# lazear/sage

Measured on NVIDIA H100. Metric: spectra/sec, higher is better.
Workload: dtype f32

## Files before the change

### sage_b200/csrc/device_common.cuh

```cuda
#pragma once
#include <cuda_runtime.h>
#include <stdint.h>

namespace sb {

constexpr int K_MAX = 128;
constexpr uint32_t NARROW_CAP = 8192;
constexpr int PRELIM_THREADS = 256;
constexpr int SCORE_THREADS = 128;
#ifndef SAGE_B200_SCORE_MIN_CTAS
#define SAGE_B200_SCORE_MIN_CTAS 10
#endif
constexpr int SCORE_MIN_CTAS = SAGE_B200_SCORE_MIN_CTAS;
#ifndef SAGE_B200_SCORE_TILE
#define SAGE_B200_SCORE_TILE 1024
#endif
#ifndef SAGE_B200_SCORE_UNROLL
#define SAGE_B200_SCORE_UNROLL 1
#endif
#ifndef SAGE_B200_SCORE_MIN_CTAS_SPLIT
#define SAGE_B200_SCORE_MIN_CTAS_SPLIT 11
#endif
constexpr int SCORE_MIN_CTAS_SPLIT = SAGE_B200_SCORE_MIN_CTAS_SPLIT;
constexpr uint32_t SCORE_UNROLL = SAGE_B200_SCORE_UNROLL;
// ... 158 lines not shown
    const uint32_t* bucket_lut;
    float blut_base, blut_inv_w;
    const uint32_t* pep_lut;
    float plut_base, plut_inv_w;
    uint64_t n_frag;
    uint8_t kinds[MAX_KINDS];
};

struct WideIndexView {
    const uint2* frag;
    const uint64_t* blk_off;
    const uint32_t* lut;
    uint32_t block, n_block, cells;
    float base, inv_w;
};

struct ScorerView {
    Tol precursor_tol, fragment_tol;
    uint32_t min_matched_peaks;
    int min_iso, max_iso;
    uint32_t min_charge, max_charge;
    int override_charge, max_fragment_charge_opt, chimera, wide_window, annotate, score_type;
    uint32_t report_psms;
    uint32_t kparam;
    uint32_t n_iso;
    uint32_t n_ch_max;
    uint32_t qmax;
    uint32_t lcap;
    uint32_t pep_cap;
    uint32_t wide_tile;
// ... 35 lines not shown
```

### sage_b200/csrc/kernels.cuh

```cuda
#pragma once
#include <type_traits>

#include "device_common.cuh"
#include "glibc_log.cuh"

#ifndef SAGE_B200_RARE_NOINLINE
#define SAGE_B200_RARE_NOINLINE 0
#endif
#if SAGE_B200_RARE_NOINLINE
#define SB_RARE __noinline__
#else
#define SB_RARE __forceinline__
#endif

namespace sb {

__device__ __forceinline__ uint32_t pep_partition(const DbView& db, float x, bool le) {
    uint32_t lo = 0, hi = db.n_pep;
    if (db.pep_lut != nullptr) {
        const float t = (x - db.plut_base) * db.plut_inv_w;
        if (t == t) {
            const int c = (int)fminf(fmaxf(floorf(t), -2.0f), (float)PEP_LUT_CELLS + 2.0f);
            lo = __ldg(db.pep_lut + min(max(c - 1, 0), (int)PEP_LUT_CELLS));
            hi = __ldg(db.pep_lut + min(max(c + 2, 0), (int)PEP_LUT_CELLS));
// ... 244 lines not shown
            const uint2 f = __ldg(&slice[e]);
            if (f.x > q.pre_hi) break;
            const float fmz = __uint_as_float(f.y);
            if (f.x >= q.eff_lo && f.x <= q.eff_hi && fmz >= flo && fmz <= fhi) {
                const uint32_t idx = f.x - q.pre_lo;
                atomicAdd(&cnt32[idx >> 1], 1u << ((idx & 1) * 16));
                matched++;
            }
        }
        pages++;
        entries += e - il;
    }
}

#ifndef SAGE_B200_WALK_SOLO
#define SAGE_B200_WALK_SOLO 8
#endif
constexpr uint32_t WALK_SOLO = SAGE_B200_WALK_SOLO;
__device__ __forceinline__ void block_probe_warp(const WideIndexView& nv, const QueryDesc& q, uint32_t b0, uint32_t b1, bool act, float flo, float fhi,
                                                 uint32_t* cnt32, uint32_t& matched) {
    const uint32_t lane = threadIdx.x & 31;
    const float tt = (flo - nv.base) * nv.inv_w;
    const int c = tt > 1.0f ? (int)fminf(tt, (float)(nv.cells - 1)) - 1 : 0;
    for (uint32_t blk = b0; blk <= b1; blk++) {
        const uint64_t base = __ldg(nv.blk_off + blk);
        const uint32_t cnt = (uint32_t)(__ldg(nv.blk_off + blk + 1) - base);
        const uint2* fr = nv.frag + base;
        uint32_t e = cnt;
        if (act) {
            e = __ldg(nv.lut + (size_t)blk * (nv.cells + 1) + c);
            for (uint32_t k = 0; k < WALK_SOLO && e < cnt; k++, e++) {
                const uint2 f = __ldg(fr + e);
                const float fmz = __uint_as_float(f.y);
                if (fmz > fhi) { e = cnt; break; }
                if (fmz >= flo && f.x >= q.eff_lo && f.x <= q.eff_hi) {
                    const uint32_t idx = f.x - q.pre_lo;
                    atomicAdd(&cnt32[idx >> 1], 1u << ((idx & 1) * 16));
                    matched++;
                }
            }
        }
        uint32_t pend = __ballot_sync(0xffffffffu, e < cnt);
        while (pend) {
            const int src = __ffs(pend) - 1;
            pend &= pend - 1;
            const uint32_t e0 = __shfl_sync(0xffffffffu, e, src);
            const float lo_s = __shfl_sync(0xffffffffu, flo, src), hi_s = __shfl_sync(0xffffffffu, fhi, src);
            for (uint32_t pos = e0; pos < cnt; pos += 32) {
                const uint32_t i = pos + lane;
                bool stop = i >= cnt;
                if (!stop) {
                    const uint2 f = __ldg(fr + i);
                    const float fmz = __uint_as_float(f.y);
                    stop = fmz > hi_s;
                    if (!stop && fmz >= lo_s && f.x >= q.eff_lo && f.x <= q.eff_hi) {
                        const uint32_t idx = f.x - q.pre_lo;
                        atomicAdd(&cnt32[idx >> 1], 1u << ((idx & 1) * 16));
                        matched++;
                    }
                }
                if (__any_sync(0xffffffffu, stop)) break;
            }
        }
    }
}

__device__ __forceinline__ void narrow_cta_query(const DbView& db, const ScorerView& sc, const BatchView& b, uint32_t pmax, uint64_t* nlist, uint32_t item,
                                                 float* bounds_smem, const WideIndexView& nv) {
    __shared__ uint32_t cnt32[NARROW_CAP / 2 + 1];
    __shared__ uint32_t s_warp[40];
    ReplaySlot* const nslots = b.nslots;
    const uint32_t s = item / sc.qmax;
    const QueryDesc q = b.queries[item];
    const uint32_t tid = threadIdx.x, lane = tid & 31, warp = tid >> 5, nwarps = PRELIM_THREADS / 32;
    const uint32_t p0 = b.peak_off[s], np = b.peak_off[s + 1] - p0;
    const uint32_t nwords = (q.potential + 1) >> 1;
    for (uint32_t i = tid; i < nwords; i += PRELIM_THREADS) cnt32[i] = 0;
    __shared__ unsigned long long s_loff;
    if (tid == 0 && q.potential > sc.kparam) s_loff = atomicAdd(b.counters + C_NLIST, (unsigned long long)q.potential);

    const uint32_t nfc = q.nfc;
    const uint32_t ntask = np * nfc;
    uint32_t my_matched = 0, my_pages = 0, my_entries = 0;
// ... 60 lines not shown
                                uint32_t bb = lut_start(LP, luts + (2 * c + 1) * LUT_CELLS, f);
                                while (bb < a && hi_c[bb] < f) bb++;
                                c_here += a - min(bb, a);
                            }
                        }
                    }
                }
                for (int o = 16; o > 0; o >>= 1) c_here += __shfl_down_sync(0xffffffffu, c_here, o);
                if (lane == 0 && c_here) {
                    const uint32_t idx = pep - q.pre_lo;
                    atomicAdd(&cnt32[idx >> 1], (c_here & 0xFFFFu) << ((idx & 1) * 16));
                    my_matched += c_here;
                }
            }
        }
    } else if (nv.frag != nullptr) {
        const uint32_t blk0 = q.pre_lo / nv.block, blk1 = min(q.pre_hi, db.n_pep - 1) / nv.block;
        for (uint32_t t0 = warp * 32; t0 < ntask; t0 += PRELIM_THREADS) {
            const uint32_t t = t0 + lane;
            const bool act = t < ntask;
            float flo = 0.0f, fhi = 0.0f;
            if (act) {
                const uint32_t p = t / nfc, fc = t - p * nfc + 1;
                const float mass = __fmul_rn(__ldg(b.masses + p0 + p), (float)fc);
                tol_bounds(sc.fragment_tol, mass, flo, fhi);
            }
            block_probe_warp(nv, q, blk0, blk1, act, flo, fhi, cnt32, my_matched);
        }
    } else {
        for (uint32_t t = tid; t < ntask; t += PRELIM_THREADS) {
            const uint32_t p = t / nfc, fc = t - p * nfc + 1;
// ... 77 lines not shown
            const uint32_t x = s_warp[w];
            if (w < warp) off += x;
            total += x;
        }
        if (c) list[wbase + off + __popc(ball & ((1u << lane) - 1))] = prescore_key(c, q.pre_lo + i, q.charge, q.iso);
        wbase += total;
        __syncthreads();
    }
    const uint32_t nzt = block_sum_u32(nzc, s_warp);
    if (tid == 0) {
        h->n = k; h->default_run = 0; h->matched_peaks = matched_total; h->scored_candidates = nzt;
        slot->off = loff; slot->item = item; slot->n_list = wbase; slot->state = 0; slot->k = k;
    }
}

__global__ void __launch_bounds__(PRELIM_THREADS) k_prelim_narrow(DbView db, ScorerView sc, BatchView b, uint32_t pmax, uint64_t* nlist, WideIndexView nv) {
    extern __shared__ float bounds_smem[];
    const uint32_t total = (uint32_t)min(b.counters[C_NCTA], (unsigned long long)b.n * sc.qmax);
    for (uint32_t i = blockIdx.x; i < total; i += gridDim.x) {
        narrow_cta_query(db, sc, b, pmax, nlist, b.cta_items[i], bounds_smem, nv);
        __syncthreads();
    }
}

template <bool BLK>
__global__ void __launch_bounds__(WARPQ_WARPS * 32, WARPQ_MIN_CTAS) k_prelim_narrow_warp(DbView db, ScorerView sc, BatchView b, uint64_t* nlist, uint32_t s_lo,
                                                                                                uint32_t s_hi, WideIndexView nv) {
    __shared__ uint32_t cnt_all[WARPQ_WARPS][WARPQ_CAP / 2];
    if (b.counters[C_COUNT + blockIdx.y] == 0ull) return;
    const uint32_t lane = threadIdx.x & 31, warp = threadIdx.x >> 5;
    const uint32_t pos = blockIdx.x * WARPQ_WARPS + warp;
    if (pos >= b.n) return;
    const uint32_t s = b.order ? b.order[pos] : pos;
    if (s < s_lo || s >= s_hi) return;
    const uint32_t item = s * sc.qmax + blockIdx.y;
    const QueryDesc q = b.queries[item];
    if (q.mode != 4) return;
    uint32_t* const cnt32 = cnt_all[warp];
    const uint32_t n = q.potential, k = min(n, sc.kparam);
    for (uint32_t i = lane; i < (n + 1) >> 1; i += 32) cnt32[i] = 0;
    unsigned long long loff = 0;
    if (n > k) {
// ... 1981 lines not shown
}
__global__ void k_wide_keys(uint64_t n_frag, const uint2* frag, uint32_t block, uint64_t* key64, uint32_t* pep) {
    const uint64_t i = (uint64_t)blockIdx.x * blockDim.x + threadIdx.x;
    if (i >= n_frag) return;
    const uint2 f = frag[i];
    key64[i] = ((uint64_t)(f.x / block) << 32) | (uint32_t)((uint32_t)f32_key(__uint_as_float(f.y)) ^ 0x80000000u);
    pep[i] = f.x;
}
__global__ void k_wide_pack(uint64_t n_frag, const uint64_t* key64, const uint32_t* pep, uint2* out) {
    const uint64_t i = (uint64_t)blockIdx.x * blockDim.x + threadIdx.x;
    if (i >= n_frag) return;
    const uint32_t u = (uint32_t)key64[i] ^ 0x80000000u;
    const uint32_t bits = u ^ (((uint32_t)((int)u >> 31)) >> 1);
    out[i] = make_uint2(pep[i], bits);
}
__global__ void k_wide_block_offsets(uint64_t n_frag, const uint64_t* key64, uint32_t n_block, uint64_t* blk_off) {
    const uint32_t b = blockIdx.x * blockDim.x + threadIdx.x;
    if (b > n_block) return;
    uint64_t lo = 0, hi = n_frag;
    const uint64_t want = (uint64_t)b << 32;
    while (lo < hi) { const uint64_t m = (lo + hi) >> 1; if (key64[m] < want) lo = m + 1; else hi = m; }
    blk_off[b] = lo;
}
__global__ void k_window_sample(DbView db, Tol ptol, uint32_t samples, unsigned long long* sum) {
    const uint32_t k = blockIdx.x * blockDim.x + threadIdx.x;
    if (k >= samples || db.n_pep == 0) return;
    const uint32_t i = (uint32_t)((uint64_t)k * db.n_pep / samples);
    float lo, hi;
    tol_bounds(ptol, __ldg(db.pep_mono + i), lo, hi);
    const uint32_t a = pep_partition(db, lo, false), b = pep_partition(db, hi, true);
    atomicAdd(sum, (unsigned long long)(b > a ? b - a : 0u));
}
__global__ void k_frag_mz_range(uint64_t n_frag, const uint2* frag, uint32_t* rng) {
    uint32_t lo = 0xFFFFFFFFu, hi = 0u;
    for (uint64_t i = (uint64_t)blockIdx.x * blockDim.x + threadIdx.x; i < n_frag; i += (uint64_t)gridDim.x * blockDim.x) {
        const uint32_t y = frag[i].y;
        lo = min(lo, y); hi = max(hi, y);
// ... 75 lines not shown
```

### sage_b200/csrc/sage_b200.cu

```cuda
#include <cub/device/device_radix_sort.cuh>
#include <cub/device/device_scan.cuh>
#include <cuda_runtime.h>

#include <pthread.h>
#include <sched.h>

#include <algorithm>
#include <atomic>
#include <cctype>
#include <cmath>
#include <cstdarg>
#include <cstdio>
#include <cstdlib>
#include <cstring>
#include <chrono>
#include <condition_variable>
#include <memory>
#include <mutex>
#include <thread>
#include <string>
#include <vector>

#include "../../include/sage_b200.h"
#include "kernels.cuh"
// ... 146 lines not shown
    const size_t nthreads = std::min<size_t>(max_threads, (size_t)hw - 1);
    const cudaError_t e = pool.run(dst, src, bytes, stage.p, piece, nthreads, st);
    if (e != cudaSuccess) return fail(SAGE_B200_ECUDA, "staged host-to-device copy failed: %s", cudaGetErrorString(e));
    return 0;
}

static bool is_pinned(const void* p) {
    cudaPointerAttributes a;
    if (cudaPointerGetAttributes(&a, p) != cudaSuccess) {
        cudaGetLastError();
        return false;
    }
    return a.type == cudaMemoryTypeHost;
}

struct BlockIndexSlot {
    WideIndexView v{};
    void *d_frag = nullptr, *d_blk = nullptr, *d_lut = nullptr;
    int failed = 0;
    uint64_t bytes = 0;
    std::vector<void*> retired;
    uint64_t retired_bytes = 0;
    void release() {
        for (void** p : {&d_frag, &d_blk, &d_lut}) { if (*p) cudaFree(*p); *p = nullptr; }
        for (void* p : retired) cudaFree(p);
        retired.clear();
        retired_bytes = 0;
        v = WideIndexView{};
        bytes = 0;
    }
    void retire() {
        for (void** p : {&d_frag, &d_blk, &d_lut}) { if (*p) retired.push_back(*p); *p = nullptr; }
        retired_bytes += bytes;
        v = WideIndexView{};
        bytes = 0;
    }
};

struct sage_b200_db {
    int device = 0;
    DbView v{};
    void *d_page_grid = nullptr, *d_bucket_lut = nullptr, *d_pep_lut = nullptr;
    void *d_frag = nullptr, *d_bucket_min = nullptr, *d_pep_mono = nullptr, *d_ion_off = nullptr, *d_ions = nullptr, *d_pep_len = nullptr,
         *d_pep_flags = nullptr, *d_pep_missed = nullptr;
    uint64_t total_residues = 0, device_bytes = 0;
    int sm_count = 132;
    mutable std::mutex wmu;
    mutable BlockIndexSlot wide, narrow;
};

static int dmalloc(sage_b200_db* db, void** p, size_t bytes) {
    if (bytes == 0) bytes = 16;
    CUDA_TRY(cudaMalloc(p, bytes));
    db->device_bytes += bytes;
    return 0;
}

static uint32_t ceil_log2_u64(uint64_t n) {
    uint32_t l = 0;
    while ((1ull << l) < n) l++;
    return l;
}

// ... 323 lines not shown
    if (nf && (fragment_peptide || fragment_mz)) {
        void *t_pep = nullptr, *t_mz = nullptr;
        CUDA_TRY(cudaMalloc(&t_pep, 4 * nf));
        CUDA_TRY(cudaMalloc(&t_mz, 4 * nf));
        k_unpack_fragments<<<(unsigned)((nf + 255) / 256), 256>>>(nf, db->v.frag, (uint32_t*)t_pep, (float*)t_mz);
        cudaError_t e = cudaDeviceSynchronize();
        if (e == cudaSuccess && fragment_peptide) e = cudaMemcpy(fragment_peptide, t_pep, 4 * nf, cudaMemcpyDeviceToHost);
        if (e == cudaSuccess && fragment_mz) e = cudaMemcpy(fragment_mz, t_mz, 4 * nf, cudaMemcpyDeviceToHost);
        cudaFree(t_pep); cudaFree(t_mz);
        if (e != cudaSuccess) return fail(SAGE_B200_ECUDA, "export failed: %s", cudaGetErrorString(e));
    }
    if (bucket_min && db->v.n_bucket) CUDA_TRY(cudaMemcpy(bucket_min, db->d_bucket_min, 4ull * db->v.n_bucket, cudaMemcpyDeviceToHost));
    return 0;
}

static WideIndexView build_block_index(const sage_b200_db* db, BlockIndexSlot& slot, uint32_t block, uint32_t cells) {
    WideIndexView none{};
    if (slot.v.frag != nullptr && slot.v.block == block) return slot.v;
    if (slot.failed || block == 0 || db->v.n_frag == 0 || db->v.n_pep == 0) return none;
    const uint64_t nf = db->v.n_frag;
    slot.retire();
    void *k_a = nullptr, *k_b = nullptr, *p_a = nullptr, *p_b = nullptr, *tmp = nullptr, *d_rng = nullptr;
    auto cleanup = [&]() { for (void* p : {k_a, k_b, p_a, p_b, tmp, d_rng}) if (p) cudaFree(p); };
    auto give_up = [&]() { cleanup(); for (void** p : {&slot.d_frag, &slot.d_blk, &slot.d_lut}) { if (*p) cudaFree(*p); *p = nullptr; } slot.v = WideIndexView{}; slot.bytes = 0; cudaGetLastError(); slot.failed = 1; return WideIndexView{}; };
    const uint32_t n_block = (db->v.n_pep + block - 1) / block;
    while (cells > 256 && (uint64_t)n_block * (cells + 1) * 4 > (1024ull << 20)) cells >>= 1;
    if (cudaMalloc(&slot.d_frag, 8 * nf + 64) != cudaSuccess || cudaMalloc(&slot.d_blk, 8 * ((size_t)n_block + 1)) != cudaSuccess ||
        cudaMalloc(&slot.d_lut, 4 * (size_t)n_block * (cells + 1)) != cudaSuccess)
        return give_up();
    if (cudaMalloc(&k_a, 8 * nf) != cudaSuccess || cudaMalloc(&k_b, 8 * nf) != cudaSuccess || cudaMalloc(&p_a, 4 * nf) != cudaSuccess ||
        cudaMalloc(&p_b, 4 * nf) != cudaSuccess || cudaMalloc(&d_rng, 8) != cudaSuccess)
        return give_up();
    k_wide_keys<<<(unsigned)((nf + 255) / 256), 256>>>(nf, db->v.frag, block, (uint64_t*)k_a, (uint32_t*)p_a);
    int nb_bits = 1;
    while (nb_bits < 32 && (n_block >> nb_bits)) nb_bits++;
    size_t tb = 0;
    if (nf > 0x7FFFFFFFull) return give_up();
    if (cub::DeviceRadixSort::SortPairs(nullptr, tb, (const uint64_t*)k_a, (uint64_t*)k_b, (const uint32_t*)p_a, (uint32_t*)p_b, (int)nf, 0, 32 + nb_bits) != cudaSuccess ||
        cudaMalloc(&tmp, tb + 16) != cudaSuccess ||
        cub::DeviceRadixSort::SortPairs(tmp, tb, (const uint64_t*)k_a, (uint64_t*)k_b, (const uint32_t*)p_a, (uint32_t*)p_b, (int)nf, 0, 32 + nb_bits) != cudaSuccess)
        return give_up();
    k_wide_pack<<<(unsigned)((nf + 255) / 256), 256>>>(nf, (const uint64_t*)k_b, (const uint32_t*)p_b, (uint2*)slot.d_frag);
    k_wide_block_offsets<<<(n_block + 1 + 255) / 256, 256>>>(nf, (const uint64_t*)k_b, n_block, (uint64_t*)slot.d_blk);
    const uint32_t rng0[2] = {0xFFFFFFFFu, 0u};
    if (cudaMemcpy(d_rng, rng0, 8, cudaMemcpyHostToDevice) != cudaSuccess) return give_up();
    k_frag_mz_range<<<(unsigned)std::min<uint64_t>((nf + 255) / 256, 4096), 256>>>(nf, db->v.frag, (uint32_t*)d_rng);
    uint32_t rng[2];
    if (cudaMemcpy(rng, d_rng, 8, cudaMemcpyDeviceToHost) != cudaSuccess) return give_up();
    cleanup();
    k_a = k_b = p_a = p_b = tmp = d_rng = nullptr;
    float lo, hi;
    memcpy(&lo, &rng[0], 4); memcpy(&hi, &rng[1], 4);
    WideIndexView w{};
    w.frag = (const uint2*)slot.d_frag; w.blk_off = (const uint64_t*)slot.d_blk; w.lut = (const uint32_t*)slot.d_lut;
    w.block = block; w.n_block = n_block; w.cells = cells;
    const float width = (hi - lo) / (float)cells;
    w.base = (std::isfinite(lo) && lo > 0.0f) ? lo : 0.0f;
    w.inv_w = (std::isfinite(width) && width > 0.0f && lo > 0.0f) ? 1.0f / width : 0.0f;
    if (w.inv_w > 0.0f) {
        const uint64_t total = (uint64_t)n_block * (cells + 1);
        k_wide_lut<<<(unsigned)((total + 255) / 256), 256>>>(w, (uint32_t*)slot.d_lut);
    } else if (cudaMemset(slot.d_lut, 0, 4 * (size_t)n_block * (cells + 1)) != cudaSuccess) return give_up();
    if (cudaDeviceSynchronize() != cudaSuccess) return give_up();
    slot.v = w;
    slot.bytes = 8 * nf + 8 * ((uint64_t)n_block + 1) + 4ull * n_block * (cells + 1);
    return w;
}

static WideIndexView db_wide_index(const sage_b200_db* db, uint32_t block) {
    std::lock_guard<std::mutex> lock(db->wmu);
    if (const char* e = getenv("SAGE_B200_NO_WIDE_INDEX")) if (e[0] == '1') return WideIndexView{};
    return build_block_index(db, db->wide, block, 1u << 18);
}

static WideIndexView db_narrow_index(const sage_b200_db* db, uint32_t block, uint32_t cells_x, bool exact) {
    std::lock_guard<std::mutex> lock(db->wmu);
    if (!exact && db->narrow.v.frag != nullptr && db->narrow.v.block * 2 >= block && db->narrow.v.block <= block * 2) return db->narrow.v;
    const uint32_t n_block = (db->v.n_pep + block - 1) / std::max(block, 1u);
    const uint64_t per_block = n_block ? db->v.n_frag / n_block : 0;
    uint32_t cells = 1024;
    while (cells < (1u << 18) && (uint64_t)cells < per_block * cells_x) cells <<= 1;
    return build_block_index(db, db->narrow, block, cells);
}

static int ensure_kernel_attributes(int device) {
    static std::mutex mu;
    static bool done[64] = {};
    std::lock_guard<std::mutex> lock(mu);
    if (device >= 0 && device < 64 && done[device]) return 0;
    int optin = 0;
    CUDA_TRY(cudaDeviceGetAttribute(&optin, cudaDevAttrMaxSharedMemoryPerBlockOptin, device));
    auto raise = [&](const void* fn) -> cudaError_t {
        cudaFuncAttributes fa;
        cudaError_t e = cudaFuncGetAttributes(&fa, fn);
        if (e != cudaSuccess) return e;
        return cudaFuncSetAttribute(fn, cudaFuncAttributeMaxDynamicSharedMemorySize, optin - (int)fa.sharedSizeBytes);
    };
// ... 115 lines not shown
    ScorerView sv{};
    std::mutex mu;
    Lane lanes[2];
    DevBuf d_lnfact, d_keep;
    uint32_t quick_mode = 0;
    int sort_spectra = 1;
    sage_b200_fragment* frag_dst = nullptr;
    uint64_t frag_cap = 0, frag_used = 0;
    int pipeline_chunks = 1;
    double nlist_per_spectrum = 512.0, wide_per_spectrum = 0.0;
    int score_split = 1;
    double hits_per_spectrum = 0.0;
    int narrow_index = 1;
    uint32_t narrow_block_auto = 0;
    int narrow_cta = 1;
    uint32_t narrow_block = 0 , narrow_cells_x = 4;
    int mass_parts = 2;
    int first_chunk_pct = 0;
    bool trace = false;
    cudaEvent_t ev_base = nullptr;
    std::chrono::steady_clock::time_point t_base;
    sage_b200_counters last{};
};

extern "C" int sage_b200_scorer_create(const sage_b200_db* db, const sage_b200_scorer_params* p, sage_b200_scorer** out) {
    if (!db || !p || !out) return fail(SAGE_B200_EINVAL, "scorer_create: null argument");
    if (p->report_psms == 0) return fail(SAGE_B200_EINVAL, "report_psms must be >= 1");
    if (p->report_psms > K_MAX / 2) return fail(SAGE_B200_ELIMIT, "report_psms %u > %d not supported", p->report_psms, K_MAX / 2);
    if (p->precursor_tol.kind < 0 || p->precursor_tol.kind > 2 || p->fragment_tol.kind < 0 || p->fragment_tol.kind > 2) return fail(SAGE_B200_EINVAL, "bad tolerance kind");
    if (p->score_type > 1) return fail(SAGE_B200_EINVAL, "bad score_type");
    CUDA_TRY(cudaSetDevice(db->device));
// ... 46 lines not shown
        CUDA_TRY(cudaStreamCreateWithFlags(&L.stream, cudaStreamNonBlocking));
        CUDA_TRY(cudaStreamCreateWithFlags(&L.copy, cudaStreamNonBlocking));
        for (auto& e : L.ev) CUDA_TRY(cudaEventCreate(&e));
        CUDA_TRY(cudaEventCreate(&L.ev_masses));
        CUDA_TRY(cudaEventCreate(&L.ev_intens));
        CUDA_TRY(cudaEventCreate(&L.ev_small));
        for (auto& e : L.ev_part) CUDA_TRY(cudaEventCreate(&e));
        CUDA_TRY(cudaStreamCreateWithFlags(&L.copy2, cudaStreamNonBlocking));
    }
    if (const char* e = getenv("SAGE_B200_PIPELINE_CHUNKS")) s->pipeline_chunks = std::max(1, atoi(e));
    if (const char* e = getenv("SAGE_B200_TRACE")) s->trace = e[0] == '1';
    if (const char* e = getenv("SAGE_B200_SCORE_SPLIT")) s->score_split = atoi(e) != 0;
    if (const char* e = getenv("SAGE_B200_NARROW_INDEX")) s->narrow_index = atoi(e) != 0;
    if (const char* e = getenv("SAGE_B200_NARROW_CTA")) s->narrow_cta = atoi(e) != 0;
    if (const char* e = getenv("SAGE_B200_NARROW_BLOCK")) s->narrow_block = (uint32_t)std::max(0, atoi(e));
    if (const char* e = getenv("SAGE_B200_NARROW_CELLS_X")) s->narrow_cells_x = (uint32_t)std::max(1, atoi(e));
    if (const char* e = getenv("SAGE_B200_MASS_PARTS")) s->mass_parts = std::min(MASS_PARTS, std::max(1, atoi(e)));
    if (const char* e = getenv("SAGE_B200_FIRST_CHUNK_PCT")) s->first_chunk_pct = std::min(50, std::max(0, atoi(e)));
    CUDA_TRY(cudaEventCreate(&s->ev_base));
    *out = s;
    return 0;
}

extern "C" int sage_b200_scorer_set_option(sage_b200_scorer* s, const char* name, int64_t value) {
    if (!s || !name) return fail(SAGE_B200_EINVAL, "scorer_set_option: null argument");
    std::lock_guard<std::mutex> lock(s->mu);
    if (!strcmp(name, "sort_spectra")) { s->sort_spectra = value != 0; return 0; }
    if (!strcmp(name, "pipeline_chunks")) { s->pipeline_chunks = (int)std::max<int64_t>(1, value); return 0; }
    if (!strcmp(name, "score_split")) { s->score_split = value != 0; return 0; }
    if (!strcmp(name, "narrow_index")) { s->narrow_index = value != 0; return 0; }
    if (!strcmp(name, "narrow_block")) {
        if (value != 0 && (value < 64 || value > (1 << 20))) return fail(SAGE_B200_EINVAL, "narrow_block must be 0 (automatic) or 64..1048576");
        s->narrow_block = (uint32_t)value;
        return 0;
    }
    if (!strcmp(name, "mass_parts")) {
        if (value < 1 || value > MASS_PARTS) return fail(SAGE_B200_EINVAL, "mass_parts must be 1..%d", MASS_PARTS);
        s->mass_parts = (int)value;
        return 0;
    }
    if (!strcmp(name, "wide_lmax")) {
        if (value < (int64_t)K_MAX || value > (int64_t)WIDE_LMAX) return fail(SAGE_B200_EINVAL, "wide_lmax must be in %d..%u", K_MAX, WIDE_LMAX);
        s->sv.wide_lmax = (uint32_t)value;
        return 0;
    }
    if (!strcmp(name, "wide_tile")) {
        if (value < 256 || value > (int64_t)WIDE_TILE || (value & 1)) return fail(SAGE_B200_EINVAL, "wide_tile must be even and in 256..%u", WIDE_TILE);
// ... 267 lines not shown
    bv.wide_cap = C.wide_cap;
    bv.nlist_cap = C.nlist_cap;
    k_setup_queries<<<(n + 127) / 128, 128, 0, st>>>(db->v, svq, bv, sk_in, sv_in);
    CUDA_TRY(cudaGetLastError());
    if (sk_in) {
        CUDA_TRY(cub::DeviceRadixSort::SortPairs(L.d_sorttmp.p, sort_tmp, sk_in, sk_out, sv_in, sv_out, (int)n, sort_lo, sort_bits, st));
        bv.order = sv_out;
    }
    CUDA_TRY(cudaEventRecord(L.ev[2], st));
    if (C.nparts <= 1) CUDA_TRY(cudaStreamWaitEvent(st, L.ev_masses, 0));
    uint64_t launches = 1;

    const size_t rsm = (size_t)sv.kparam * REPLAY_THREADS * 8;
    const float ptol_span = std::max(std::fabs(sv.precursor_tol.lo), std::fabs(sv.precursor_tol.hi));
    const bool narrow_tol = ptol_span <= (sv.precursor_tol.kind == 0 ? 2000.0f : sv.precursor_tol.kind == 1 ? 0.2f : 5.0f);
    WideIndexView nv{};
    if (S->narrow_index && !sv.wide_window && narrow_tol) {
        if (S->narrow_block == 0 && (rc = narrow_block_for(S))) return rc;
        nv = db_narrow_index(db, S->narrow_block ? S->narrow_block : S->narrow_block_auto, S->narrow_cells_x, S->narrow_block != 0);
    }
    for (uint32_t q = 0; q < C.nparts; q++) {
        if (C.nparts > 1) CUDA_TRY(cudaStreamWaitEvent(st, L.ev_part[q], 0));
        const dim3 wgrid((n + WARPQ_WARPS - 1) / WARPQ_WARPS, sv.qmax);
        if (nv.frag != nullptr) k_prelim_narrow_warp<true><<<wgrid, WARPQ_WARPS * 32, 0, st>>>(db->v, svq, bv, L.d_nlist.as<uint64_t>(), C.part_lo[q], C.part_lo[q + 1], nv);
        else k_prelim_narrow_warp<false><<<wgrid, WARPQ_WARPS * 32, 0, st>>>(db->v, svq, bv, L.d_nlist.as<uint64_t>(), C.part_lo[q], C.part_lo[q + 1], nv);
        CUDA_TRY(cudaGetLastError());
        launches += q > 0;
    }
    if (C.nparts > 1) CUDA_TRY(cudaStreamWaitEvent(st, L.ev_masses, 0));
    k_prelim_narrow<<<(unsigned)std::min<uint64_t>(C.nitems, (uint64_t)db->sm_count * 6), PRELIM_THREADS, pep_smem, st>>>(db->v, svq, bv, C.pmax, L.d_nlist.as<uint64_t>(),
                                                                                                                         S->narrow_cta ? nv : WideIndexView{});
    CUDA_TRY(cudaGetLastError());
    CUDA_TRY(cudaEventRecord(L.ev[8], st));
    k_replay<true><<<(unsigned)((C.nitems + REPLAY_THREADS - 1) / REPLAY_THREADS), REPLAY_THREADS, rsm / 2, st>>>(sv, bv, L.d_nlist.as<uint64_t>(), L.d_nslots.as<ReplaySlot>(),
                                                                                                                 (uint32_t)C.nitems, nullptr, n);
    CUDA_TRY(cudaGetLastError());
    launches += 3;
    if (C.wide_cap) {
        const int ctas = (int)std::min<uint64_t>((uint64_t)db->sm_count * WIDE_CTAS, C.wide_cap);
        const WideIndexView wv = db_wide_index(db, sv.wide_tile);
        k_prelim_wide<<<ctas, WIDE_THREADS, sizeof(WideSmem), st>>>(db->v, sv, bv, (uint32_t)C.nitems, L.d_wlist.as<uint64_t>(), L.d_wslots.as<WideSlot>(), wv);
        CUDA_TRY(cudaGetLastError());
        if (wv.frag != nullptr) {
            k_wide_account<<<(C.wide_cap + 7) / 8, 256, 0, st>>>(db->v, sv, bv);
            CUDA_TRY(cudaGetLastError());
            launches++;
// ... 685 lines not shown
```

Baseline: 23.15 million.

## Split narrow fragment index into SoA m/z and 16-bit peptide offsets with per-block grid

Result: faster. 24.38 million, median of 6 (+5.3%).

```diff
diff --git a/sage_b200/csrc/device_common.cuh b/sage_b200/csrc/device_common.cuh
--- a/sage_b200/csrc/device_common.cuh
+++ b/sage_b200/csrc/device_common.cuh
@@ -196,6 +196,19 @@
     uint32_t block, n_block, cells;
     float base, inv_w;
 };
+
+struct NarrowIndexView {
+    const float* mz;
+    const uint16_t* pep;
+    const uint32_t* blk_off;
+    const uint16_t* dir;
+    const float2* grid;
+    uint32_t block, n_block, cells, shift;
+};
+__device__ __forceinline__ uint32_t narrow_cell(float2 grid, uint32_t cells, float x) {
+    const float t = __fmul_rn(__fsub_rn(x, grid.x), grid.y);
+    return t >= (float)cells ? cells : (t > 0.0f ? (uint32_t)t : 0u);
+}
 
 struct ScorerView {
     Tol precursor_tol, fragment_tol;
diff --git a/sage_b200/csrc/kernels.cuh b/sage_b200/csrc/kernels.cuh
--- a/sage_b200/csrc/kernels.cuh
+++ b/sage_b200/csrc/kernels.cuh
@@ -282,51 +282,54 @@
 }
 
 #ifndef SAGE_B200_WALK_SOLO
-#define SAGE_B200_WALK_SOLO 8
+#define SAGE_B200_WALK_SOLO 2
 #endif
 constexpr uint32_t WALK_SOLO = SAGE_B200_WALK_SOLO;
-__device__ __forceinline__ void block_probe_warp(const WideIndexView& nv, const QueryDesc& q, uint32_t b0, uint32_t b1, bool act, float flo, float fhi,
+__device__ __forceinline__ void narrow_count(const QueryDesc& q, uint32_t pid, uint32_t* cnt32, uint32_t& matched) {
+    if (pid >= q.eff_lo && pid <= q.eff_hi) {
+        const uint32_t idx = pid - q.pre_lo;
+        atomicAdd(&cnt32[idx >> 1], 1u << ((idx & 1) * 16));
+        matched++;
+    }
+}
+__device__ __forceinline__ void block_probe_warp(const NarrowIndexView& nv, const QueryDesc& q, uint32_t b0, uint32_t b1, bool act, float flo, float fhi,
                                                  uint32_t* cnt32, uint32_t& matched) {
     const uint32_t lane = threadIdx.x & 31;
-    const float tt = (flo - nv.base) * nv.inv_w;
-    const int c = tt > 1.0f ? (int)fminf(tt, (float)(nv.cells - 1)) - 1 : 0;
     for (uint32_t blk = b0; blk <= b1; blk++) {
-        const uint64_t base = __ldg(nv.blk_off + blk);
-        const uint32_t cnt = (uint32_t)(__ldg(nv.blk_off + blk + 1) - base);
-        const uint2* fr = nv.frag + base;
-        uint32_t e = cnt;
+        const uint32_t end = __ldg(nv.blk_off + blk + 1);
+        uint32_t e = end;
         if (act) {
-            e = __ldg(nv.lut + (size_t)blk * (nv.cells + 1) + c);
-            for (uint32_t k = 0; k < WALK_SOLO && e < cnt; k++, e++) {
-                const uint2 f = __ldg(fr + e);
-                const float fmz = __uint_as_float(f.y);
-                if (fmz > fhi) { e = cnt; break; }
-                if (fmz >= flo && f.x >= q.eff_lo && f.x <= q.eff_hi) {
-                    const uint32_t idx = f.x - q.pre_lo;
-                    atomicAdd(&cnt32[idx >> 1], 1u << ((idx & 1) * 16));
-                    matched++;
-                }
-            }
-        }
-        uint32_t pend = __ballot_sync(0xffffffffu, e < cnt);
+            const uint32_t c = narrow_cell(__ldg(nv.grid + blk), nv.cells, flo);
+            const uint32_t g = __ldg(nv.blk_off + blk) + ((uint32_t)__ldg(nv.dir + (size_t)blk * (nv.cells + 1) + c) << nv.shift);
+            const uint32_t a = g & ~3u;
+            float v[4 * WALK_SOLO];
+#pragma unroll
+            for (uint32_t k = 0; k < WALK_SOLO; k++) {
+                const float4 x = __ldg(reinterpret_cast<const float4*>(nv.mz + a) + k);
+                v[4 * k] = x.x; v[4 * k + 1] = x.y; v[4 * k + 2] = x.z; v[4 * k + 3] = x.w;
+            }
+            e = a + 4 * WALK_SOLO;
+#pragma unroll
+            for (uint32_t j = 0; j < 4 * WALK_SOLO; j++) {
+                const uint32_t i = a + j;
+                if (i < g) continue;
+                if (i >= end || v[j] > fhi) { e = end; break; }
+                if (v[j] >= flo) narrow_count(q, blk * nv.block + __ldg(nv.pep + i), cnt32, matched);
+            }
+        }
+        uint32_t pend = __ballot_sync(0xffffffffu, e < end);
         while (pend) {
             const int src = __ffs(pend) - 1;
             pend &= pend - 1;
             const uint32_t e0 = __shfl_sync(0xffffffffu, e, src);
             const float lo_s = __shfl_sync(0xffffffffu, flo, src), hi_s = __shfl_sync(0xffffffffu, fhi, src);
-            for (uint32_t pos = e0; pos < cnt; pos += 32) {
+            for (uint32_t pos = e0; pos < end; pos += 32) {
                 const uint32_t i = pos + lane;
-                bool stop = i >= cnt;
-                if (!stop) {
-                    const uint2 f = __ldg(fr + i);
-                    const float fmz = __uint_as_float(f.y);
-                    stop = fmz > hi_s;
-                    if (!stop && fmz >= lo_s && f.x >= q.eff_lo && f.x <= q.eff_hi) {
-                        const uint32_t idx = f.x - q.pre_lo;
-                        atomicAdd(&cnt32[idx >> 1], 1u << ((idx & 1) * 16));
-                        matched++;
-                    }
-                }
+                const bool in = i < end;
+                const float m = in ? __ldg(nv.mz + i) : 0.0f;
+                const uint32_t off = in ? __ldg(nv.pep + i) : 0u;
+                const bool stop = !in || m > hi_s;
+                if (!stop && m >= lo_s) narrow_count(q, blk * nv.block + off, cnt32, matched);
                 if (__any_sync(0xffffffffu, stop)) break;
             }
         }
@@ -334,7 +337,7 @@
 }
 
 __device__ __forceinline__ void narrow_cta_query(const DbView& db, const ScorerView& sc, const BatchView& b, uint32_t pmax, uint64_t* nlist, uint32_t item,
-                                                 float* bounds_smem, const WideIndexView& nv) {
+                                                 float* bounds_smem, const NarrowIndexView& nv) {
     __shared__ uint32_t cnt32[NARROW_CAP / 2 + 1];
     __shared__ uint32_t s_warp[40];
     ReplaySlot* const nslots = b.nslots;
@@ -425,7 +428,7 @@
                 }
             }
         }
-    } else if (nv.frag != nullptr) {
+    } else if (nv.mz != nullptr) {
         const uint32_t blk0 = q.pre_lo / nv.block, blk1 = min(q.pre_hi, db.n_pep - 1) / nv.block;
         for (uint32_t t0 = warp * 32; t0 < ntask; t0 += PRELIM_THREADS) {
             const uint32_t t = t0 + lane;
@@ -533,7 +536,7 @@
     }
 }
 
-__global__ void __launch_bounds__(PRELIM_THREADS) k_prelim_narrow(DbView db, ScorerView sc, BatchView b, uint32_t pmax, uint64_t* nlist, WideIndexView nv) {
+__global__ void __launch_bounds__(PRELIM_THREADS) k_prelim_narrow(DbView db, ScorerView sc, BatchView b, uint32_t pmax, uint64_t* nlist, NarrowIndexView nv) {
     extern __shared__ float bounds_smem[];
     const uint32_t total = (uint32_t)min(b.counters[C_NCTA], (unsigned long long)b.n * sc.qmax);
     for (uint32_t i = blockIdx.x; i < total; i += gridDim.x) {
@@ -544,7 +547,7 @@
 
 template <bool BLK>
 __global__ void __launch_bounds__(WARPQ_WARPS * 32, WARPQ_MIN_CTAS) k_prelim_narrow_warp(DbView db, ScorerView sc, BatchView b, uint64_t* nlist, uint32_t s_lo,
-                                                                                                uint32_t s_hi, WideIndexView nv) {
+                                                                                                uint32_t s_hi, NarrowIndexView nv) {
     __shared__ uint32_t cnt_all[WARPQ_WARPS][WARPQ_CAP / 2];
     if (b.counters[C_COUNT + blockIdx.y] == 0ull) return;
     const uint32_t lane = threadIdx.x & 31, warp = threadIdx.x >> 5;
@@ -2556,13 +2559,50 @@
     const uint32_t bits = u ^ (((uint32_t)((int)u >> 31)) >> 1);
     out[i] = make_uint2(pep[i], bits);
 }
-__global__ void k_wide_block_offsets(uint64_t n_frag, const uint64_t* key64, uint32_t n_block, uint64_t* blk_off) {
+template <class Off>
+__global__ void k_wide_block_offsets(uint64_t n_frag, const uint64_t* key64, uint32_t n_block, Off* blk_off) {
     const uint32_t b = blockIdx.x * blockDim.x + threadIdx.x;
     if (b > n_block) return;
     uint64_t lo = 0, hi = n_frag;
     const uint64_t want = (uint64_t)b << 32;
     while (lo < hi) { const uint64_t m = (lo + hi) >> 1; if (key64[m] < want) lo = m + 1; else hi = m; }
-    blk_off[b] = lo;
+    blk_off[b] = (Off)lo;
+}
+__global__ void k_narrow_pack(uint64_t n_frag, const uint64_t* key64, const uint32_t* pep, uint32_t block, float* mz, uint16_t* pep_off) {
+    const uint64_t i = (uint64_t)blockIdx.x * blockDim.x + threadIdx.x;
+    if (i >= n_frag) return;
+    const uint64_t k = key64[i];
+    const uint32_t u = (uint32_t)k ^ 0x80000000u;
+    mz[i] = __uint_as_float(u ^ (((uint32_t)((int)u >> 31)) >> 1));
+    pep_off[i] = (uint16_t)(pep[i] - (uint32_t)(k >> 32) * block);
+}
+__global__ void k_narrow_grid(uint32_t n_block, const float* mz, const uint32_t* blk_off, uint32_t cells, float2* grid) {
+    const uint32_t b = blockIdx.x * blockDim.x + threadIdx.x;
+    if (b >= n_block) return;
+    float lo = 0.0f, inv_w = 0.0f;
+    if (blk_off[b + 1] > blk_off[b]) {
+        lo = mz[blk_off[b]];
+        const float width = __fdiv_rn(__fsub_rn(mz[blk_off[b + 1] - 1], lo), (float)cells);
+        if (isfinite(lo) && lo > 0.0f && isfinite(width) && width > 0.0f) inv_w = __fdiv_rn(1.0f, width);
+        else lo = 0.0f;
+    }
+    grid[b] = make_float2(lo, inv_w);
+}
+__global__ void k_narrow_dir(NarrowIndexView nv, uint16_t* dir) {
+    const uint64_t j = (uint64_t)blockIdx.x * blockDim.x + threadIdx.x;
+    const uint64_t per = (uint64_t)nv.cells + 1;
+    if (j >= (uint64_t)nv.n_block * per) return;
+    const uint32_t b = (uint32_t)(j / per), c = (uint32_t)(j - (uint64_t)b * per);
+    const float* m = nv.mz + nv.blk_off[b];
+    const float2 grid = nv.grid[b];
+    uint32_t lo = 0, hi = nv.blk_off[b + 1] - nv.blk_off[b];
+    while (lo < hi) {
+        const uint32_t mid = (lo + hi) >> 1;
+        const float x = m[mid];
+        const uint32_t cx = x != x ? (signbit(x) ? 0u : nv.cells + 1) : narrow_cell(grid, nv.cells, x);
+        if (cx < c) lo = mid + 1; else hi = mid;
+    }
+    dir[j] = (uint16_t)(lo >> nv.shift);
 }
 __global__ void k_window_sample(DbView db, Tol ptol, uint32_t samples, unsigned long long* sum) {
     const uint32_t k = blockIdx.x * blockDim.x + threadIdx.x;
diff --git a/sage_b200/csrc/sage_b200.cu b/sage_b200/csrc/sage_b200.cu
--- a/sage_b200/csrc/sage_b200.cu
+++ b/sage_b200/csrc/sage_b200.cu
@@ -184,26 +184,35 @@
     return a.type == cudaMemoryTypeHost;
 }
 
+template <class View>
 struct BlockIndexSlot {
-    WideIndexView v{};
-    void *d_frag = nullptr, *d_blk = nullptr, *d_lut = nullptr;
+    View v{};
+    void* d[5] = {};
     int failed = 0;
     uint64_t bytes = 0;
     std::vector<void*> retired;
     uint64_t retired_bytes = 0;
     void release() {
-        for (void** p : {&d_frag, &d_blk, &d_lut}) { if (*p) cudaFree(*p); *p = nullptr; }
+        for (void*& p : d) { if (p) cudaFree(p); p = nullptr; }
         for (void* p : retired) cudaFree(p);
         retired.clear();
         retired_bytes = 0;
-        v = WideIndexView{};
+        v = View{};
         bytes = 0;
     }
     void retire() {
-        for (void** p : {&d_frag, &d_blk, &d_lut}) { if (*p) retired.push_back(*p); *p = nullptr; }
+        for (void*& p : d) { if (p) retired.push_back(p); p = nullptr; }
         retired_bytes += bytes;
-        v = WideIndexView{};
+        v = View{};
         bytes = 0;
+    }
+    View give_up() {
+        for (void*& p : d) { if (p) cudaFree(p); p = nullptr; }
+        v = View{};
+        bytes = 0;
+        cudaGetLastError();
+        failed = 1;
+        return View{};
     }
 };
 
@@ -216,7 +225,8 @@
     uint64_t total_residues = 0, device_bytes = 0;
     int sm_count = 132;
     mutable std::mutex wmu;
-    mutable BlockIndexSlot wide, narrow;
+    mutable BlockIndexSlot<WideIndexView> wide;
+    mutable BlockIndexSlot<NarrowIndexView> narrow;
 };
 
 static int dmalloc(sage_b200_db* db, void** p, size_t bytes) {
@@ -570,54 +580,73 @@
     return 0;
 }
 
-static WideIndexView build_block_index(const sage_b200_db* db, BlockIndexSlot& slot, uint32_t block, uint32_t cells) {
-    WideIndexView none{};
-    if (slot.v.frag != nullptr && slot.v.block == block) return slot.v;
-    if (slot.failed || block == 0 || db->v.n_frag == 0 || db->v.n_pep == 0) return none;
+static bool sort_block_keys(const sage_b200_db* db, uint32_t block, uint32_t n_block, void** keys, void** peps) {
     const uint64_t nf = db->v.n_frag;
-    slot.retire();
-    void *k_a = nullptr, *k_b = nullptr, *p_a = nullptr, *p_b = nullptr, *tmp = nullptr, *d_rng = nullptr;
-    auto cleanup = [&]() { for (void* p : {k_a, k_b, p_a, p_b, tmp, d_rng}) if (p) cudaFree(p); };
-    auto give_up = [&]() { cleanup(); for (void** p : {&slot.d_frag, &slot.d_blk, &slot.d_lut}) { if (*p) cudaFree(*p); *p = nullptr; } slot.v = WideIndexView{}; slot.bytes = 0; cudaGetLastError(); slot.failed = 1; return WideIndexView{}; };
-    const uint32_t n_block = (db->v.n_pep + block - 1) / block;
-    while (cells > 256 && (uint64_t)n_block * (cells + 1) * 4 > (1024ull << 20)) cells >>= 1;
-    if (cudaMalloc(&slot.d_frag, 8 * nf + 64) != cudaSuccess || cudaMalloc(&slot.d_blk, 8 * ((size_t)n_block + 1)) != cudaSuccess ||
-        cudaMalloc(&slot.d_lut, 4 * (size_t)n_block * (cells + 1)) != cudaSuccess)
-        return give_up();
+    void *k_a = nullptr, *k_b = nullptr, *p_a = nullptr, *p_b = nullptr, *tmp = nullptr;
+    auto fail_ = [&]() { for (void* p : {k_a, k_b, p_a, p_b, tmp}) if (p) cudaFree(p); return false; };
+    if (nf > 0x7FFFFFFFull) return false;
     if (cudaMalloc(&k_a, 8 * nf) != cudaSuccess || cudaMalloc(&k_b, 8 * nf) != cudaSuccess || cudaMalloc(&p_a, 4 * nf) != cudaSuccess ||
-        cudaMalloc(&p_b, 4 * nf) != cudaSuccess || cudaMalloc(&d_rng, 8) != cudaSuccess)
-        return give_up();
+        cudaMalloc(&p_b, 4 * nf) != cudaSuccess)
+        return fail_();
     k_wide_keys<<<(unsigned)((nf + 255) / 256), 256>>>(nf, db->v.frag, block, (uint64_t*)k_a, (uint32_t*)p_a);
     int nb_bits = 1;
     while (nb_bits < 32 && (n_block >> nb_bits)) nb_bits++;
     size_t tb = 0;
-    if (nf > 0x7FFFFFFFull) return give_up();
     if (cub::DeviceRadixSort::SortPairs(nullptr, tb, (const uint64_t*)k_a, (uint64_t*)k_b, (const uint32_t*)p_a, (uint32_t*)p_b, (int)nf, 0, 32 + nb_bits) != cudaSuccess ||
         cudaMalloc(&tmp, tb + 16) != cudaSuccess ||
-        cub::DeviceRadixSort::SortPairs(tmp, tb, (const uint64_t*)k_a, (uint64_t*)k_b, (const uint32_t*)p_a, (uint32_t*)p_b, (int)nf, 0, 32 + nb_bits) != cudaSuccess)
-        return give_up();
-    k_wide_pack<<<(unsigned)((nf + 255) / 256), 256>>>(nf, (const uint64_t*)k_b, (const uint32_t*)p_b, (uint2*)slot.d_frag);
-    k_wide_block_offsets<<<(n_block + 1 + 255) / 256, 256>>>(nf, (const uint64_t*)k_b, n_block, (uint64_t*)slot.d_blk);
+        cub::DeviceRadixSort::SortPairs(tmp, tb, (const uint64_t*)k_a, (uint64_t*)k_b, (const uint32_t*)p_a, (uint32_t*)p_b, (int)nf, 0, 32 + nb_bits) != cudaSuccess ||
+        cudaDeviceSynchronize() != cudaSuccess)
+        return fail_();
+    cudaFree(k_a); cudaFree(p_a); cudaFree(tmp);
+    *keys = k_b; *peps = p_b;
+    return true;
+}
+
+static bool frag_mz_grid(const sage_b200_db* db, uint32_t cells, float& base, float& inv_w) {
+    const uint64_t nf = db->v.n_frag;
+    void* d_rng = nullptr;
     const uint32_t rng0[2] = {0xFFFFFFFFu, 0u};
-    if (cudaMemcpy(d_rng, rng0, 8, cudaMemcpyHostToDevice) != cudaSuccess) return give_up();
-    k_frag_mz_range<<<(unsigned)std::min<uint64_t>((nf + 255) / 256, 4096), 256>>>(nf, db->v.frag, (uint32_t*)d_rng);
     uint32_t rng[2];
-    if (cudaMemcpy(rng, d_rng, 8, cudaMemcpyDeviceToHost) != cudaSuccess) return give_up();
-    cleanup();
-    k_a = k_b = p_a = p_b = tmp = d_rng = nullptr;
+    bool ok = cudaMalloc(&d_rng, 8) == cudaSuccess && cudaMemcpy(d_rng, rng0, 8, cudaMemcpyHostToDevice) == cudaSuccess;
+    if (ok) {
+        k_frag_mz_range<<<(unsigned)std::min<uint64_t>((nf + 255) / 256, 4096), 256>>>(nf, db->v.frag, (uint32_t*)d_rng);
+        ok = cudaMemcpy(rng, d_rng, 8, cudaMemcpyDeviceToHost) == cudaSuccess;
+    }
+    if (d_rng) cudaFree(d_rng);
+    if (!ok) return false;
     float lo, hi;
     memcpy(&lo, &rng[0], 4); memcpy(&hi, &rng[1], 4);
+    const float width = (hi - lo) / (float)cells;
+    base = (std::isfinite(lo) && lo > 0.0f) ? lo : 0.0f;
+    inv_w = (std::isfinite(width) && width > 0.0f && lo > 0.0f) ? 1.0f / width : 0.0f;
+    return true;
+}
+
+static WideIndexView build_block_index(const sage_b200_db* db, BlockIndexSlot<WideIndexView>& slot, uint32_t block, uint32_t cells) {
+    if (slot.v.frag != nullptr && slot.v.block == block) return slot.v;
+    if (slot.failed || block == 0 || db->v.n_frag == 0 || db->v.n_pep == 0) return WideIndexView{};
+    const uint64_t nf = db->v.n_frag;
+    slot.retire();
+    const uint32_t n_block = (db->v.n_pep + block - 1) / block;
+    while (cells > 256 && (uint64_t)n_block * (cells + 1) * 4 > (1024ull << 20)) cells >>= 1;
+    if (cudaMalloc(&slot.d[0], 8 * nf + 64) != cudaSuccess || cudaMalloc(&slot.d[1], 8 * ((size_t)n_block + 1)) != cudaSuccess ||
+        cudaMalloc(&slot.d[2], 4 * (size_t)n_block * (cells + 1)) != cudaSuccess)
+        return slot.give_up();
+    void *keys = nullptr, *peps = nullptr;
+    if (!sort_block_keys(db, block, n_block, &keys, &peps)) return slot.give_up();
+    k_wide_pack<<<(unsigned)((nf + 255) / 256), 256>>>(nf, (const uint64_t*)keys, (const uint32_t*)peps, (uint2*)slot.d[0]);
+    k_wide_block_offsets<<<(n_block + 1 + 255) / 256, 256>>>(nf, (const uint64_t*)keys, n_block, (uint64_t*)slot.d[1]);
+    const bool synced = cudaDeviceSynchronize() == cudaSuccess;
+    cudaFree(keys); cudaFree(peps);
     WideIndexView w{};
-    w.frag = (const uint2*)slot.d_frag; w.blk_off = (const uint64_t*)slot.d_blk; w.lut = (const uint32_t*)slot.d_lut;
+    if (!synced || !frag_mz_grid(db, cells, w.base, w.inv_w)) return slot.give_up();
+    w.frag = (const uint2*)slot.d[0]; w.blk_off = (const uint64_t*)slot.d[1]; w.lut = (const uint32_t*)slot.d[2];
     w.block = block; w.n_block = n_block; w.cells = cells;
-    const float width = (hi - lo) / (float)cells;
-    w.base = (std::isfinite(lo) && lo > 0.0f) ? lo : 0.0f;
-    w.inv_w = (std::isfinite(width) && width > 0.0f && lo > 0.0f) ? 1.0f / width : 0.0f;
     if (w.inv_w > 0.0f) {
         const uint64_t total = (uint64_t)n_block * (cells + 1);
-        k_wide_lut<<<(unsigned)((total + 255) / 256), 256>>>(w, (uint32_t*)slot.d_lut);
-    } else if (cudaMemset(slot.d_lut, 0, 4 * (size_t)n_block * (cells + 1)) != cudaSuccess) return give_up();
-    if (cudaDeviceSynchronize() != cudaSuccess) return give_up();
+        k_wide_lut<<<(unsigned)((total + 255) / 256), 256>>>(w, (uint32_t*)slot.d[2]);
+    } else if (cudaMemset(slot.d[2], 0, 4 * (size_t)n_block * (cells + 1)) != cudaSuccess) return slot.give_up();
+    if (cudaDeviceSynchronize() != cudaSuccess) return slot.give_up();
     slot.v = w;
     slot.bytes = 8 * nf + 8 * ((uint64_t)n_block + 1) + 4ull * n_block * (cells + 1);
     return w;
@@ -629,14 +658,54 @@
     return build_block_index(db, db->wide, block, 1u << 18);
 }
 
-static WideIndexView db_narrow_index(const sage_b200_db* db, uint32_t block, uint32_t cells_x, bool exact) {
+#ifndef SAGE_B200_NARROW_PER_CELL
+#define SAGE_B200_NARROW_PER_CELL 1
+#endif
+constexpr uint32_t NARROW_PER_CELL = SAGE_B200_NARROW_PER_CELL;
+
+static NarrowIndexView build_narrow_index(const sage_b200_db* db, BlockIndexSlot<NarrowIndexView>& slot, uint32_t block) {
+    if (slot.v.mz != nullptr && slot.v.block == block) return slot.v;
+    if (slot.failed || block == 0 || block > 65536 || db->v.n_frag == 0 || db->v.n_pep == 0) return NarrowIndexView{};
+    const uint64_t nf = db->v.n_frag;
+    slot.retire();
+    const uint32_t n_block = (db->v.n_pep + block - 1) / block;
+    uint32_t cells = 256;
+    while (cells < (1u << 20) && (uint64_t)cells * NARROW_PER_CELL < nf / n_block) cells <<= 1;
+    while (cells > 256 && (uint64_t)n_block * (cells + 1) * 2 > (1024ull << 20)) cells >>= 1;
+    const size_t dir_n = (size_t)n_block * (cells + 1);
+    if (cudaMalloc(&slot.d[0], 4 * (nf + 8)) != cudaSuccess || cudaMalloc(&slot.d[1], 2 * nf) != cudaSuccess ||
+        cudaMalloc(&slot.d[2], 4 * ((size_t)n_block + 1)) != cudaSuccess || cudaMalloc(&slot.d[3], 2 * dir_n) != cudaSuccess ||
+        cudaMalloc(&slot.d[4], 8 * (size_t)n_block) != cudaSuccess ||
+        cudaMemset((float*)slot.d[0] + nf, 0, 32) != cudaSuccess)
+        return slot.give_up();
+    void *keys = nullptr, *peps = nullptr;
+    if (!sort_block_keys(db, block, n_block, &keys, &peps)) return slot.give_up();
+    k_narrow_pack<<<(unsigned)((nf + 255) / 256), 256>>>(nf, (const uint64_t*)keys, (const uint32_t*)peps, block, (float*)slot.d[0], (uint16_t*)slot.d[1]);
+    k_wide_block_offsets<<<(n_block + 1 + 255) / 256, 256>>>(nf, (const uint64_t*)keys, n_block, (uint32_t*)slot.d[2]);
+    const bool synced = cudaDeviceSynchronize() == cudaSuccess;
+    cudaFree(keys); cudaFree(peps);
+    NarrowIndexView v{};
+    if (!synced) return slot.give_up();
+    k_narrow_grid<<<(n_block + 255) / 256, 256>>>(n_block, (const float*)slot.d[0], (const uint32_t*)slot.d[2], cells, (float2*)slot.d[4]);
+    std::vector<uint32_t> off((size_t)n_block + 1);
+    if (cudaMemcpy(off.data(), slot.d[2], 4 * off.size(), cudaMemcpyDeviceToHost) != cudaSuccess) return slot.give_up();
+    uint32_t most = 0;
+    for (uint32_t b = 0; b < n_block; b++) most = std::max(most, off[b + 1] - off[b]);
+    while ((most >> v.shift) > 0xFFFFu) v.shift++;
+    v.mz = (const float*)slot.d[0]; v.pep = (const uint16_t*)slot.d[1]; v.blk_off = (const uint32_t*)slot.d[2]; v.dir = (const uint16_t*)slot.d[3];
+    v.grid = (const float2*)slot.d[4];
+    v.block = block; v.n_block = n_block; v.cells = cells;
+    k_narrow_dir<<<(unsigned)((dir_n + 255) / 256), 256>>>(v, (uint16_t*)slot.d[3]);
+    if (cudaDeviceSynchronize() != cudaSuccess) return slot.give_up();
+    slot.v = v;
+    slot.bytes = 4 * (nf + 8) + 2 * nf + 4 * ((uint64_t)n_block + 1) + 2ull * dir_n + 8ull * n_block;
+    return v;
+}
+
+static NarrowIndexView db_narrow_index(const sage_b200_db* db, uint32_t block, bool exact) {
     std::lock_guard<std::mutex> lock(db->wmu);
-    if (!exact && db->narrow.v.frag != nullptr && db->narrow.v.block * 2 >= block && db->narrow.v.block <= block * 2) return db->narrow.v;
-    const uint32_t n_block = (db->v.n_pep + block - 1) / std::max(block, 1u);
-    const uint64_t per_block = n_block ? db->v.n_frag / n_block : 0;
-    uint32_t cells = 1024;
-    while (cells < (1u << 18) && (uint64_t)cells < per_block * cells_x) cells <<= 1;
-    return build_block_index(db, db->narrow, block, cells);
+    if (!exact && db->narrow.v.mz != nullptr && db->narrow.v.block * 2 >= block && db->narrow.v.block <= block * 2) return db->narrow.v;
+    return build_narrow_index(db, db->narrow, block);
 }
 
 static int ensure_kernel_attributes(int device) {
@@ -782,7 +851,7 @@
     int narrow_index = 1;
     uint32_t narrow_block_auto = 0;
     int narrow_cta = 1;
-    uint32_t narrow_block = 0 , narrow_cells_x = 4;
+    uint32_t narrow_block = 0;
     int mass_parts = 2;
     int first_chunk_pct = 0;
     bool trace = false;
@@ -859,7 +928,6 @@
     if (const char* e = getenv("SAGE_B200_NARROW_INDEX")) s->narrow_index = atoi(e) != 0;
     if (const char* e = getenv("SAGE_B200_NARROW_CTA")) s->narrow_cta = atoi(e) != 0;
     if (const char* e = getenv("SAGE_B200_NARROW_BLOCK")) s->narrow_block = (uint32_t)std::max(0, atoi(e));
-    if (const char* e = getenv("SAGE_B200_NARROW_CELLS_X")) s->narrow_cells_x = (uint32_t)std::max(1, atoi(e));
     if (const char* e = getenv("SAGE_B200_MASS_PARTS")) s->mass_parts = std::min(MASS_PARTS, std::max(1, atoi(e)));
     if (const char* e = getenv("SAGE_B200_FIRST_CHUNK_PCT")) s->first_chunk_pct = std::min(50, std::max(0, atoi(e)));
     CUDA_TRY(cudaEventCreate(&s->ev_base));
@@ -875,7 +943,7 @@
     if (!strcmp(name, "score_split")) { s->score_split = value != 0; return 0; }
     if (!strcmp(name, "narrow_index")) { s->narrow_index = value != 0; return 0; }
     if (!strcmp(name, "narrow_block")) {
-        if (value != 0 && (value < 64 || value > (1 << 20))) return fail(SAGE_B200_EINVAL, "narrow_block must be 0 (automatic) or 64..1048576");
+        if (value != 0 && (value < 64 || value > 65536)) return fail(SAGE_B200_EINVAL, "narrow_block must be 0 (automatic) or 64..65536");
         s->narrow_block = (uint32_t)value;
         return 0;
     }
@@ -1173,22 +1241,22 @@
     const size_t rsm = (size_t)sv.kparam * REPLAY_THREADS * 8;
     const float ptol_span = std::max(std::fabs(sv.precursor_tol.lo), std::fabs(sv.precursor_tol.hi));
     const bool narrow_tol = ptol_span <= (sv.precursor_tol.kind == 0 ? 2000.0f : sv.precursor_tol.kind == 1 ? 0.2f : 5.0f);
-    WideIndexView nv{};
+    NarrowIndexView nv{};
     if (S->narrow_index && !sv.wide_window && narrow_tol) {
         if (S->narrow_block == 0 && (rc = narrow_block_for(S))) return rc;
-        nv = db_narrow_index(db, S->narrow_block ? S->narrow_block : S->narrow_block_auto, S->narrow_cells_x, S->narrow_block != 0);
+        nv = db_narrow_index(db, S->narrow_block ? S->narrow_block : S->narrow_block_auto, S->narrow_block != 0);
     }
     for (uint32_t q = 0; q < C.nparts; q++) {
         if (C.nparts > 1) CUDA_TRY(cudaStreamWaitEvent(st, L.ev_part[q], 0));
         const dim3 wgrid((n + WARPQ_WARPS - 1) / WARPQ_WARPS, sv.qmax);
-        if (nv.frag != nullptr) k_prelim_narrow_warp<true><<<wgrid, WARPQ_WARPS * 32, 0, st>>>(db->v, svq, bv, L.d_nlist.as<uint64_t>(), C.part_lo[q], C.part_lo[q + 1], nv);
+        if (nv.mz != nullptr) k_prelim_narrow_warp<true><<<wgrid, WARPQ_WARPS * 32, 0, st>>>(db->v, svq, bv, L.d_nlist.as<uint64_t>(), C.part_lo[q], C.part_lo[q + 1], nv);
         else k_prelim_narrow_warp<false><<<wgrid, WARPQ_WARPS * 32, 0, st>>>(db->v, svq, bv, L.d_nlist.as<uint64_t>(), C.part_lo[q], C.part_lo[q + 1], nv);
         CUDA_TRY(cudaGetLastError());
         launches += q > 0;
     }
     if (C.nparts > 1) CUDA_TRY(cudaStreamWaitEvent(st, L.ev_masses, 0));
     k_prelim_narrow<<<(unsigned)std::min<uint64_t>(C.nitems, (uint64_t)db->sm_count * 6), PRELIM_THREADS, pep_smem, st>>>(db->v, svq, bv, C.pmax, L.d_nlist.as<uint64_t>(),
-                                                                                                                         S->narrow_cta ? nv : WideIndexView{});
+                                                                                                                         S->narrow_cta ? nv : NarrowIndexView{});
     CUDA_TRY(cudaGetLastError());
     CUDA_TRY(cudaEventRecord(L.ev[8], st));
     k_replay<true><<<(unsigned)((C.nitems + REPLAY_THREADS - 1) / REPLAY_THREADS), REPLAY_THREADS, rsm / 2, st>>>(sv, bv, L.d_nlist.as<uint64_t>(), L.d_nslots.as<ReplaySlot>(),
```
